# beehive-lab/GPULlama3.java

Measured on AMD Instinct MI355X. Metric: tg128 tok/s (llama-bench), Llama-3-8B Q8_0, higher is better.
Workload: dtype i8; 1 GPU; Llama-3-8B-random Q8_0 random-weight GGUF-layout model, tg128 at depth 0 (one step = 128 decode tokens, logits D2H inside the timed region); parallelism=single GPU, ranks=1, ctx=648

## Files before the change

### gpullama3.java_amd/csrc/gl3_decode_kernels.h

```cpp
#pragma once
#include <hip/hip_runtime.h>
#include <stdint.h>

#include "gl3_seqsum.h"

namespace gl3 {

constexpr int TILE_BYTES = 2176;
constexpr int MV_AUX = 4;
__host__ __device__ constexpr int mv_threads(int npw) { return 64 * (npw + MV_AUX); }

enum { PRO_RMS = 0, PRO_QUANT = 1 };
enum { EPI_STORE = 0, EPI_RESID = 1, EPI_SWIGLU = 2 };

typedef float v4f __attribute__((ext_vector_type(4)));

#ifdef GL3_MV_TIMING
__device__ long long gl3_mv_stamp[32];
#define ATT_STAMP(i) do { if (blockIdx.x == 0 && threadIdx.x == 0) gl3_mv_stamp[i] = wall_clock64(); } while (0)
#define MV_STAMP(i, cond) do { if (blockIdx.x == 0 && (cond)) gl3_mv_stamp[i] = clock64(); } while (0)
#define PV_T(...) __VA_ARGS__
#else
#define PV_T(...)
#define MV_STAMP(i, cond)
#define ATT_STAMP(i)
#endif

constexpr int TPF_MAX_PEERS = 15;
struct TpWait {
    const uint32_t* flags;
    const uint32_t* step;
    uint32_t* err;
    int mul, add, tp, me;
    unsigned spin_limit;
};
struct TpPush {
    uint32_t* ticket;
    const uint32_t* step;
    int mul, add, npeers;
    long delta[TPF_MAX_PEERS];
    uint32_t* flag[TPF_MAX_PEERS];
};
struct TpRec { TpWait w; TpPush p; };

__device__ __forceinline__ void tp_wait(const TpWait& w) {
    const uint32_t need = (__hip_atomic_load(w.step, __ATOMIC_RELAXED, __HIP_MEMORY_SCOPE_AGENT) - 1u) * (uint32_t)w.mul + (uint32_t)w.add;
    const int lane = threadIdx.x & 63;
    const bool mine = lane < w.tp && lane != w.me;
    unsigned spins = 0;
    for (;;) {
        const bool ok = !mine || (int32_t)(__hip_atomic_load(w.flags + (mine ? lane : 0), __ATOMIC_RELAXED, __HIP_MEMORY_SCOPE_SYSTEM) - need) >= 0;
        if (__builtin_amdgcn_ballot_w64(!ok) == 0) break;
        __builtin_amdgcn_s_sleep(8);
        if (++spins > w.spin_limit) { if (lane == 0) __hip_atomic_store(w.err, 1u, __ATOMIC_RELAXED, __HIP_MEMORY_SCOPE_SYSTEM); break; }
    }
    __builtin_amdgcn_fence(__ATOMIC_ACQUIRE, "");
}
__device__ __forceinline__ void tp_push_store(const TpPush& p, float* own, float v) {
    for (int j = 0; j < p.npeers; ++j)
        *reinterpret_cast<float*>(reinterpret_cast<uint8_t*>(own) + p.delta[j]) = v;
}
__device__ __forceinline__ void tp_publish(const TpPush& p, unsigned total) {
    asm volatile("s_waitcnt vmcnt(0)" ::: "memory");
    if ((threadIdx.x & 63) != 0) return;
    const unsigned ticket = __hip_atomic_fetch_add(p.ticket, 1u, __ATOMIC_RELAXED, __HIP_MEMORY_SCOPE_AGENT);
    if (ticket != total - 1) return;
    __hip_atomic_store(p.ticket, 0u, __ATOMIC_RELAXED, __HIP_MEMORY_SCOPE_AGENT);
    const uint32_t k = (__hip_atomic_load(p.step, __ATOMIC_RELAXED, __HIP_MEMORY_SCOPE_AGENT) - 1u) * (uint32_t)p.mul + (uint32_t)p.add;
    __threadfence_system();
    for (int j = 0; j < p.npeers; ++j) __hip_atomic_store(p.flag[j], k, __ATOMIC_RELEASE, __HIP_MEMORY_SCOPE_SYSTEM);
}

static __global__ __launch_bounds__(64) void tp_wait_kernel(const TpRec* r) { tp_wait(r->w); }

struct MatvecArgs {
    const uint8_t* w;
    const uint8_t* w2;
    int rows;
    int k;
    int ng;
    int nstrips;
    const float* x;
    const float* norm_w;
    float eps;
    float* out;
    const float* resid_in;
    float out_scale;
    const struct MoeSlots* moe;
    const TpRec* tp;
};

struct MoeSlots {
    const int* sel;
    size_t sel_stride;
    int x_slot_stride, out_slot_stride;
    int n_sel, sh_rows;
    const uint8_t* sh_w;
    const uint8_t* sh_w2;
    float* sh_out;
};

__device__ __forceinline__ void lds_barrier() { asm volatile("s_waitcnt lgkmcnt(0)\n\ts_barrier" ::: "memory"); }

struct LdsBarrier { __device__ __forceinline__ void operator()() const { lds_barrier(); } };

__device__ __forceinline__ float h2f(uint16_t h) { return (float)__builtin_bit_cast(_Float16, h); }

__device__ __forceinline__ float wave_max(float v) {
#pragma unroll
    for (int m = 32; m >= 1; m >>= 1) v = fmaxf(v, __shfl_xor(v, m, 64));
    return v;
}

template <bool SQ>
__device__ __forceinline__ float seq_add4(float s, const float4& a) {
    if (SQ) { s = s + a.x * a.x; s = s + a.y * a.y; s = s + a.z * a.z; s = s + a.w * a.w; }
    else { s = s + a.x; s = s + a.y; s = s + a.z; s = s + a.w; }
    return s;
}
template <bool SQ>
__device__ __forceinline__ float seq_sum_lds(const float* v, int n, float start = 0.f) {
    float s = start;
    int i = 0;
    if (n >= 16) {
        float4 a0 = *reinterpret_cast<const float4*>(v), a1 = *reinterpret_cast<const float4*>(v + 4);
        for (; i + 16 <= n; i += 8) {
            const float4 b0 = *reinterpret_cast<const float4*>(v + i + 8), b1 = *reinterpret_cast<const float4*>(v + i + 12);
            s = seq_add4<SQ>(s, a0); s = seq_add4<SQ>(s, a1);
            a0 = b0; a1 = b1;
        }
        s = seq_add4<SQ>(s, a0); s = seq_add4<SQ>(s, a1);
        i += 8;
    }
    for (; i + 4 <= n; i += 4) s = seq_add4<SQ>(s, *reinterpret_cast<const float4*>(v + i));
    for (; i < n; ++i) s = SQ ? s + v[i] * v[i] : s + v[i];
    return s;
}

__device__ __forceinline__ float mul_f32_scalar(float a, float b) {
    float r;
    asm("v_mul_f32 %0, %1, %2" : "=v"(r) : "v"(a), "v"(b));
    return r;
}

__device__ __forceinline__ float seq_sum_lds_ring(const float* v, int n, float start = 0.f) {
    float s = start;
    const int G = n >> 4;
    int i = 0;
    if (G >= 3) {
        float4 a0, a1, a2, a3, b0, b1, b2, b3, c0, c1, c2, c3;
#define SSR_LD(G_, V0_, V1_, V2_, V3_) do { const float* q_ = v + 16 * min((G_), G - 1); V0_ = *reinterpret_cast<const float4*>(q_); \
        V1_ = *reinterpret_cast<const float4*>(q_ + 4); V2_ = *reinterpret_cast<const float4*>(q_ + 8); V3_ = *reinterpret_cast<const float4*>(q_ + 12); } while (0)
#define SSR_ADD(V0_, V1_, V2_, V3_) do { s = seq_add4<false>(s, V0_); s = seq_add4<false>(s, V1_); s = seq_add4<false>(s, V2_); s = seq_add4<false>(s, V3_); } while (0)
        SSR_LD(0, a0, a1, a2, a3); SSR_LD(1, b0, b1, b2, b3); SSR_LD(2, c0, c1, c2, c3);
        int g = 0;
        for (; g + 3 <= G; g += 3) {
            SSR_ADD(a0, a1, a2, a3); SSR_LD(g + 3, a0, a1, a2, a3); __builtin_amdgcn_sched_barrier(0);
            SSR_ADD(b0, b1, b2, b3); SSR_LD(g + 4, b0, b1, b2, b3); __builtin_amdgcn_sched_barrier(0);
            SSR_ADD(c0, c1, c2, c3); SSR_LD(g + 5, c0, c1, c2, c3); __builtin_amdgcn_sched_barrier(0);
        }
        if (g < G) { SSR_ADD(a0, a1, a2, a3); ++g; }
        if (g < G) { SSR_ADD(b0, b1, b2, b3); ++g; }
#undef SSR_ADD
#undef SSR_LD
        i = 16 * G;
    }
    for (; i + 4 <= n; i += 4) s = seq_add4<false>(s, *reinterpret_cast<const float4*>(v + i));
    for (; i < n; ++i) s = s + v[i];
    return s;
}

__device__ __forceinline__ uint32_t quantize_quad_pack(float4 v, float& qs_out) {
    float amax = fmaxf(fmaxf(fabsf(v.x), fabsf(v.y)), fmaxf(fabsf(v.z), fabsf(v.w)));
    amax = fmaxf(amax, __builtin_bit_cast(float, __builtin_amdgcn_update_dpp(0, __builtin_bit_cast(int, amax), 0xB1, 0xf, 0xf, false)));
    amax = fmaxf(amax, __builtin_bit_cast(float, __builtin_amdgcn_update_dpp(0, __builtin_bit_cast(int, amax), 0x4E, 0xf, 0xf, false)));
    amax = fmaxf(amax, __builtin_bit_cast(float, __builtin_amdgcn_update_dpp(0, __builtin_bit_cast(int, amax), 0x141, 0xf, 0xf, false)));
    const float qs = amax / 127.0f;
    const float ainv = qs != 0.f ? 1.0f / qs : 0.f;
    const float s0 = v.x * ainv, s1 = v.y * ainv, s2 = v.z * ainv, s3 = v.w * ainv;
    const int q0 = (int)(s0 + copysignf(0.5f, s0)), q1 = (int)(s1 + copysignf(0.5f, s1));
    const int q2 = (int)(s2 + copysignf(0.5f, s2)), q3 = (int)(s3 + copysignf(0.5f, s3));
    qs_out = (float)(_Float16)qs;
    return (uint32_t)(q0 & 0xFF) | ((uint32_t)(q1 & 0xFF) << 8) | ((uint32_t)(q2 & 0xFF) << 16) | ((uint32_t)(q3 & 0xFF) << 24);
}

__device__ __forceinline__ void quantize_quad(float4 v, int qd, uint8_t* xq, float* xs) {
    float qs;
    const uint32_t packed = quantize_quad_pack(v, qs);
    *reinterpret_cast<uint32_t*>(xq + 4 * qd) = packed;
    if ((qd & 7) == 0) xs[qd >> 3] = qs;
}

__device__ __forceinline__ size_t bdq_offset(int qd, int tok, int tslots) {
    const int blk = qd >> 3, qi = qd & 7, c = qi >> 1;
    const int g = ((c & 1) << 1) | (c >> 1);
    return ((size_t)(blk >> 1) * tslots + tok) * 64 + 16 * g + 8 * (blk & 1) + 4 * (qi & 1);
}
__device__ __forceinline__ size_t bds_offset(int blk, int tok, int tslots) { return ((size_t)(blk >> 2) * tslots + tok) * 4 + (blk & 3); }

__device__ __forceinline__ int dot32(const int4& a0, const int4& a1, const int4& b0, const int4& b1) {
    int s = 0;
    s = __builtin_amdgcn_sdot4(a0.x, b0.x, s, false); s = __builtin_amdgcn_sdot4(a0.y, b0.y, s, false);
    s = __builtin_amdgcn_sdot4(a0.z, b0.z, s, false); s = __builtin_amdgcn_sdot4(a0.w, b0.w, s, false);
    s = __builtin_amdgcn_sdot4(a1.x, b1.x, s, false); s = __builtin_amdgcn_sdot4(a1.y, b1.y, s, false);
    s = __builtin_amdgcn_sdot4(a1.z, b1.z, s, false); s = __builtin_amdgcn_sdot4(a1.w, b1.w, s, false);
    return s;
}

template <bool NT>
__device__ __forceinline__ int4 ld16(const uint8_t* p) {
    typedef int v4i __attribute__((ext_vector_type(4)));
    v4i v;
    if (NT) v = __builtin_nontemporal_load(reinterpret_cast<const v4i*>(p));
    else v = *reinterpret_cast<const v4i*>(p);
    int4 r; r.x = v.x; r.y = v.y; r.z = v.z; r.w = v.w;
    return r;
}
template <bool NT>
__device__ __forceinline__ uint16_t ld2(const uint8_t* p) {
    if (NT) return __builtin_nontemporal_load(reinterpret_cast<const uint16_t*>(p));
    return *reinterpret_cast<const uint16_t*>(p);
}

template <int PRO, int EPI, bool NT, int NPW = 4, bool SEL = false, bool TPF = false>
__global__ __launch_bounds__(mv_threads(NPW), NPW == 4 ? 4 : 2) void matvec_q8t_kernel(const MatvecArgs a_in) {
    MatvecArgs a = a_in;
    if (SEL) {
        const int slot = blockIdx.y;
        const MoeSlots m = *a.moe;
        if (slot < m.n_sel) {
            const size_t woff = (size_t)m.sel[slot] * m.sel_stride;
            a.w += woff;
            if (a.w2) a.w2 += woff;
            a.x += (size_t)slot * m.x_slot_stride;
            a.out += (size_t)slot * m.out_slot_stride;
        } else {
            const int c = slot - m.n_sel;
            const size_t woff = (size_t)c * m.sel_stride;
            a.w = m.sh_w + woff;
            a.w2 = m.sh_w2 ? m.sh_w2 + woff : nullptr;
            a.out = m.sh_out + (size_t)c * a.rows;
            const int left = m.sh_rows - c * a.rows;
            if (left < a.rows) { a.rows = left; a.nstrips = (left + 15) / 16; }
        }
    }
    constexpr int MV_PRODUCERS = NPW;
    extern __shared__ __attribute__((aligned(16))) uint8_t smem[];
    constexpr int NM = (EPI == EPI_SWIGLU) ? 2 : 1;
    constexpr int CH = (NM == 1) ? 8 : 4;
    const int t = threadIdx.x, lane = t & 63, wave = t >> 6;
    const int nb4 = a.ng * 4;
    uint8_t* xq = smem;
    float* xs = reinterpret_cast<float*>(smem + (size_t)nb4 * 32);
    float* xf = xs + nb4;
    float* pbuf = xf + (PRO == PRO_RMS ? a.k + 32 : 0);
    float* red = pbuf + (size_t)2 * NM * a.ng * 64;
    int* sync_w = reinterpret_cast<int*>(red + 4);
    const size_t strip_bytes = (size_t)a.ng * TILE_BYTES;
    MV_STAMP(0, t == 0);
    if (t < 2) sync_w[t] = 0;

    if (wave < MV_PRODUCERS) {
        const int nt = (a.ng - wave + MV_PRODUCERS - 1) / MV_PRODUCERS;
        uint16_t sc[NM][CH];
        int4 lo[NM][CH], hi[NM][CH];
        auto issue = [&](int strip, int i0) {
#pragma unroll
            for (int u = 0; u < CH; ++u) {
                if (i0 + u < nt) {
                    const int g = wave + (i0 + u) * MV_PRODUCERS;
#pragma unroll
                    for (int m = 0; m < NM; ++m) {
                        const uint8_t* p = (m == 0 ? a.w : a.w2) + (size_t)strip * strip_bytes + (size_t)g * TILE_BYTES;
                        sc[m][u] = ld2<NT>(p + 2 * lane);
                        lo[m][u] = ld16<NT>(p + 128 + 16 * lane);
                        hi[m][u] = ld16<NT>(p + 1152 + 16 * lane);
                    }
                }
            }
        };
        auto compute = [&](int i0, float* pb) {
#pragma unroll
            for (int u = 0; u < CH; ++u) {
                if (i0 + u < nt) {
                    const int g = wave + (i0 + u) * MV_PRODUCERS;
                    const int xb = 4 * g + (lane >> 4);
                    const int4 xlo = *reinterpret_cast<const int4*>(xq + 32 * xb);
                    const int4 xhi = *reinterpret_cast<const int4*>(xq + 32 * xb + 16);
                    const float xsc = xs[xb];
#pragma unroll
                    for (int m = 0; m < NM; ++m) {
                        const int isum = dot32(lo[m][u], hi[m][u], xlo, xhi);
                        pb[(size_t)m * a.ng * 64 + g * 64 + lane] = (float)isum * (h2f(sc[m][u]) * xsc);
                    }
                }
            }
        };
        int strip = blockIdx.x;
        __syncthreads();
        if (strip < a.nstrips) issue(strip, 0);
        while (__hip_atomic_load(&sync_w[1], __ATOMIC_RELAXED, __HIP_MEMORY_SCOPE_WORKGROUP) == 0) __builtin_amdgcn_s_sleep(2);
        __builtin_amdgcn_fence(__ATOMIC_ACQUIRE, "workgroup");
        MV_STAMP(3, t == 0);
        int it = 0;
        for (; strip < a.nstrips; strip += gridDim.x, ++it) {
            float* pb = pbuf + (size_t)(it & 1) * NM * a.ng * 64;
            for (int i0 = 0; i0 < nt; i0 += CH) {
                if (it != 0 || i0 != 0) issue(strip, i0);
                compute(i0, pb);
            }
            MV_STAMP(4 + 2 * it, t == 0 && it < 4);
            __syncthreads();
            MV_STAMP(5 + 2 * it, t == 0 && it < 4);
        }
        return;
    }

    __builtin_amdgcn_s_setprio(3);
    const int ta = t - 64 * MV_PRODUCERS;
    const int nquads = a.k >> 2;
    float scale = 1.0f;
    constexpr int NXV = (PRO == PRO_RMS) ? 5 : 14;
    float4 nwv[5], xv[NXV];
    if (!TPF) {
#pragma unroll
        for (int i = 0; i < NXV; ++i) xv[i] = *reinterpret_cast<const float4*>(a.x + 4 * min(ta + 256 * i, nquads - 1));
    }
    if (PRO == PRO_RMS) {
#pragma unroll
        for (int i = 0; i < 5; ++i) nwv[i] = *reinterpret_cast<const float4*>(a.norm_w + 4 * min(ta + 256 * i, nquads - 1));
    }
    __syncthreads();
    if (TPF) {
        if (a.tp->w.flags) tp_wait(a.tp->w);
#pragma unroll
        for (int i = 0; i < NXV; ++i) xv[i] = *reinterpret_cast<const float4*>(a.x + 4 * min(ta + 256 * i, nquads - 1));
    }
    SubBarrier aux_sync{&sync_w[0], MV_AUX, 0};
    if (PRO == PRO_RMS) {
        if (nquads <= NXV * 256) {
#pragma unroll
            for (int i = 0; i < NXV; ++i) { const int qd = ta + 256 * i; if (qd < nquads) *reinterpret_cast<float4*>(xf + 4 * qd) = xv[i]; }
        } else {
            for (int qd = ta; qd < nquads; qd += 256)
                *reinterpret_cast<float4*>(xf + 4 * qd) = *reinterpret_cast<const float4*>(a.x + 4 * qd);
        }
        if (ta < 32) xf[a.k + ta] = 0.f;
        aux_sync();
        MV_STAMP(1, ta == 0);
        float ss;
        if ((size_t)2 * NM * a.ng * 64 * 4 >= ss_scratch_bytes(a.k) && a.k >= 1024 && a.k <= 5120) {
            ss = exact_sumsq_lds(xf, a.k, reinterpret_cast<uint8_t*>(pbuf), ta, aux_sync);
        } else {
            if (wave == MV_PRODUCERS) {
                const float s1 = seq_sum_lds<true>(xf, a.k);
                if (lane == 0) red[0] = s1;
            }
            aux_sync();
            ss = red[0];
        }
        MV_STAMP(2, ta == 0);
        ss /= (float)a.k;
        ss += a.eps;
        scale = (float)(1.0 / sqrt((double)ss));
    }
    for (int b = (a.k >> 5) + ta; b < nb4; b += 256) {
        xs[b] = 0.f;
        const int4 z = {0, 0, 0, 0};
        *reinterpret_cast<int4*>(xq + 32 * b) = z;
        *reinterpret_cast<int4*>(xq + 32 * b + 16) = z;
    }
    if (nquads <= NXV * 256) {
#pragma unroll
        for (int i = 0; i < NXV; ++i) {
            const int qd = ta + 256 * i;
            if (qd < nquads) {
                float4 v = xv[i];
                if (PRO == PRO_RMS) {
                    const float4 w = nwv[i];
                    v.x = w.x * (scale * v.x); v.y = w.y * (scale * v.y); v.z = w.z * (scale * v.z); v.w = w.w * (scale * v.w);
                }
                quantize_quad(v, qd, xq, xs);
            }
        }
    } else {
        for (int qd = ta; qd < nquads; qd += 256) {
            float4 v = *reinterpret_cast<const float4*>(a.x + 4 * qd);
            if (PRO == PRO_RMS) {
                const float4 w = *reinterpret_cast<const float4*>(a.norm_w + 4 * qd);
                v.x = w.x * (scale * v.x); v.y = w.y * (scale * v.y); v.z = w.z * (scale * v.z); v.w = w.w * (scale * v.w);
            }
            quantize_quad(v, qd, xq, xs);
        }
    }
    aux_sync();
    if (ta == 0) __hip_atomic_store(&sync_w[1], 1, __ATOMIC_RELEASE, __HIP_MEMORY_SCOPE_WORKGROUP);
    if (wave != MV_PRODUCERS) return;

    int it = 0;
    for (int strip = blockIdx.x; strip < a.nstrips; strip += gridDim.x, ++it) {
        __syncthreads();
        MV_STAMP(16 + 2 * it, lane == 0 && it < 4);
        const float* pb = pbuf + (size_t)(it & 1) * NM * a.ng * 64;
        v4f acc[NM];
#pragma unroll
        for (int m = 0; m < NM; ++m) acc[m] = (v4f){0.f, 0.f, 0.f, 0.f};
        int g = 0;
        for (; g + 8 <= a.ng; g += 8) {
            float av[NM][8];
#pragma unroll
            for (int m = 0; m < NM; ++m)
#pragma unroll
                for (int u = 0; u < 8; ++u) av[m][u] = pb[(size_t)m * a.ng * 64 + (g + u) * 64 + lane];
#pragma unroll
            for (int u = 0; u < 8; ++u)
#pragma unroll
                for (int m = 0; m < NM; ++m) acc[m] = __builtin_amdgcn_mfma_f32_16x16x4f32(av[m][u], 1.0f, acc[m], 0, 0, 0);
        }
        for (; g < a.ng; ++g)
#pragma unroll
            for (int m = 0; m < NM; ++m)
                acc[m] = __builtin_amdgcn_mfma_f32_16x16x4f32(pb[(size_t)m * a.ng * 64 + g * 64 + lane], 1.0f, acc[m], 0, 0, 0);
        MV_STAMP(17 + 2 * it, lane == 0 && it < 4);
        if ((lane & 15) < 4) {
            const int r = lane & 3;
            const int row = strip * 16 + 4 * (lane >> 4) + r;
            if (row < a.rows) {
                const float v0 = r == 0 ? acc[0][0] : r == 1 ? acc[0][1] : r == 2 ? acc[0][2] : acc[0][3];
                float res;
                if (EPI == EPI_STORE) res = v0 * a.out_scale;
                if (EPI == EPI_RESID) res = a.resid_in ? a.resid_in[row] + v0 * a.out_scale : v0 * a.out_scale;
                if (EPI == EPI_SWIGLU) {
                    const float v1 = r == 0 ? acc[NM - 1][0] : r == 1 ? acc[NM - 1][1] : r == 2 ? acc[NM - 1][2] : acc[NM - 1][3];
                    const float gte = v0 / (float)(1.0 + exp(-(double)v0));
                    res = gte * v1;
                }
                a.out[row] = res;
                if (TPF) tp_push_store(a.tp->p, a.out + row, res);
            }
        }
    }
    if (TPF && a.tp->p.npeers) tp_publish(a.tp->p, gridDim.x);
}

static __global__ __launch_bounds__(256) void embed_q8t_kernel(const uint8_t* __restrict__ emb, int ng, int dim,
                                                         const int* __restrict__ dyn, float* __restrict__ x, float emb_scale,
                                                         const TpRec* tp = nullptr, uint32_t* step = nullptr) {
    if (step) {
        const uint32_t s = *step;
        __syncthreads();
        if (threadIdx.x == 0) *step = s + 1;
        if (tp) {
            TpWait w = tp->w;
            const uint32_t need = s * (uint32_t)w.mul;
            const int lane = threadIdx.x & 63;
            const bool mine = lane < w.tp && lane != w.me;
            unsigned spins = 0;
            for (;;) {
                const bool ok = !mine || (int32_t)(__hip_atomic_load(w.flags + (mine ? lane : 0), __ATOMIC_RELAXED, __HIP_MEMORY_SCOPE_SYSTEM) - need) >= 0;
                if (__builtin_amdgcn_ballot_w64(!ok) == 0) break;
                __builtin_amdgcn_s_sleep(8);
                if (++spins > w.spin_limit) { if (lane == 0) __hip_atomic_store(w.err, 1u, __ATOMIC_RELAXED, __HIP_MEMORY_SCOPE_SYSTEM); break; }
            }
        }
    }
    const int token = dyn[0];
    const uint8_t* strip = emb + (size_t)(token >> 4) * ng * TILE_BYTES;
    const int i16 = token & 15;
    for (int i = threadIdx.x; i < dim; i += 256) {
        const int b = i >> 5, j = i & 31;
        const uint8_t* p = strip + (size_t)(b >> 2) * TILE_BYTES;
        const int l = i16 + 16 * (b & 3);
        const float d = h2f(*reinterpret_cast<const uint16_t*>(p + 2 * l));
        const int8_t q = (int8_t)p[(j < 16 ? 128 : 1152) + 16 * l + (j & 15)];
        x[i] = ((float)q * d) * emb_scale;
    }
}

struct AttnArgs {
    const float* qkv;
    float* kcache;
    float* vcache;
    const float* rope_cr;
    const float* rope_ci;
    const float* qnorm;
    const float* knorm;
    const float* bq;
    const float* bk;
    const float* bv;
    const int* dyn;
    float* att;
    float* xb;
    int n_heads, n_kv_heads, hs, q_dim, kv_dim, ctx;
    float eps;
    int arch;
    const int* seqv;
    const int* posv;
    size_t seq_stride;
    int qkv_stride, xb_stride;
    float att_mul;
    int win;
    int att_stride;
    float* att_t;
    float* tmax;
    float* sums;
    int group;
    uint8_t* xq_out; float* xs_out; int xq_slots;
    const TpRec* tp;
};

__device__ __forceinline__ void rope_head(float* v, int hs, const float* cr, const float* ci, int arch, int t0, int nthreads) {
    const int half = hs >> 1;
    for (int i = t0; i < half; i += nthreads) {
        const float fcr = cr[i], fci = ci[i];
        const int i0 = arch == 0 ? 2 * i : i, i1 = arch == 0 ? 2 * i + 1 : i + half;
        const float v0 = v[i0], v1 = v[i1];
        v[i0] = v0 * fcr - v1 * fci;
        v[i1] = v0 * fci + v1 * fcr;
    }
}

__device__ __forceinline__ void head_rmsnorm_wave(float* v, const float* __restrict__ w, int hs, float eps, int lane) {
    float ss = seq_sum_lds<true>(v, hs);
    ss /= (float)hs;
    ss += eps;
    ss = (float)(1.0 / sqrt((double)ss));
    for (int i = lane; i < hs; i += 64) v[i] = w[i] * (ss * v[i]);
}

constexpr int ATT_TT = 64;

static __global__ void attn_scores_kernel(const AttnArgs a) {
    extern __shared__ __attribute__((aligned(16))) float sm[];
    const int hs = a.hs, kvmul = a.n_heads / a.n_kv_heads, half = hs >> 1;
    float* q_s = sm;
    float* kt = q_s + kvmul * hs;
    float* cr_s = kt + ATT_TT * (hs + 4);
    float* ci_s = cr_s + half;
    const int t = threadIdx.x, nthr = blockDim.x;
    const int sp = blockIdx.x, kvh = blockIdx.y;
    const int pos = a.dyn[1];
    const int t0 = sp * ATT_TT;
    if (t0 > pos) return;
    const int t1 = min(pos + 1, t0 + ATT_TT);
    const bool owns_pos = (t1 == pos + 1);
    const int pitch = hs + 4;
    float* krow = kt + (pos - t0) * pitch;
    const int q4 = hs >> 2;
    const int nrows_cache = owns_pos ? (t1 - 1 - t0) : (t1 - t0);
    const int nk4 = nrows_cache * q4;
    constexpr int KMAX = 16;
    float4 kreg[KMAX];
    const int per = (nk4 + nthr - 1) / nthr;
#pragma unroll
    for (int u = 0; u < KMAX; ++u) {
        kreg[u] = make_float4(0.f, 0.f, 0.f, 0.f);
        if (u < per) {
            const int i = min(t + u * nthr, nk4 - 1);
            kreg[u] = *reinterpret_cast<const float4*>(a.kcache + (size_t)(t0 + i / q4) * a.kv_dim + kvh * hs + 4 * (i % q4));
        }
    }
    for (int i = t; i < kvmul * hs; i += nthr) q_s[i] = a.bq ? a.qkv[(kvh * kvmul) * hs + i] + a.bq[(kvh * kvmul) * hs + i] : a.qkv[(kvh * kvmul) * hs + i];
    for (int i = t; i < half; i += nthr) { cr_s[i] = a.rope_cr[(size_t)pos * half + i]; ci_s[i] = a.rope_ci[(size_t)pos * half + i]; }
    float vraw[4] = {0.f, 0.f, 0.f, 0.f};
    if (owns_pos) {
        for (int i = t; i < hs; i += nthr) krow[i] = a.bk ? a.qkv[a.q_dim + kvh * hs + i] + a.bk[kvh * hs + i] : a.qkv[a.q_dim + kvh * hs + i];
#pragma unroll
        for (int u = 0; u < 4; ++u) {
            const int i = t + u * nthr;
            if (i < hs) vraw[u] = a.bv ? a.qkv[a.q_dim + a.kv_dim + kvh * hs + i] + a.bv[kvh * hs + i] : a.qkv[a.q_dim + a.kv_dim + kvh * hs + i];
        }
    }
    if (per > KMAX) {
        for (int i = t; i < nk4; i += nthr) {
            const float4 v = *reinterpret_cast<const float4*>(a.kcache + (size_t)(t0 + i / q4) * a.kv_dim + kvh * hs + 4 * (i % q4));
            *reinterpret_cast<float4*>(kt + (i / q4) * pitch + 4 * (i % q4)) = v;
        }
    } else {
#pragma unroll
        for (int u = 0; u < KMAX; ++u) {
            const int i = t + u * nthr;
            if (u < per && i < nk4) *reinterpret_cast<float4*>(kt + (i / q4) * pitch + 4 * (i % q4)) = kreg[u];
        }
    }
    __syncthreads();
    if (a.arch == 1) {
        const int nvec = kvmul + (owns_pos ? 1 : 0);
        for (int vec = t >> 6; vec < nvec; vec += nthr >> 6)
            head_rmsnorm_wave(vec < kvmul ? q_s + vec * hs : krow, vec < kvmul ? a.qnorm : a.knorm, hs, a.eps, t & 63);
        __syncthreads();
    }
    for (int h = 0; h < kvmul; ++h) rope_head(q_s + h * hs, hs, cr_s, ci_s, a.arch, t, nthr);
    if (owns_pos) rope_head(krow, hs, cr_s, ci_s, a.arch, t, nthr);
    __syncthreads();
    if (owns_pos) {
#pragma unroll
        for (int u = 0; u < 4; ++u) {
            const int i = t + u * nthr;
            if (i < hs) {
                a.kcache[(size_t)pos * a.kv_dim + kvh * hs + i] = krow[i];
                a.vcache[(size_t)pos * a.kv_dim + kvh * hs + i] = vraw[u];
            }
        }
    }
    const int hq = t >> 6, r = t & 63;
    float my_score = -INFINITY;
    if (hq < kvmul && t0 + r < t1) {
        const float* q = q_s + hq * hs;
        const float* kk = kt + r * pitch;
        float score = 0.f;
        float4 qv = *reinterpret_cast<const float4*>(q), kv = *reinterpret_cast<const float4*>(kk);
        for (int j = 4; j < hs; j += 4) {
            const float4 qn = *reinterpret_cast<const float4*>(q + j), kn = *reinterpret_cast<const float4*>(kk + j);
            score = score + qv.x * kv.x; score = score + qv.y * kv.y; score = score + qv.z * kv.z; score = score + qv.w * kv.w;
            qv = qn; kv = kn;
        }
        score = score + qv.x * kv.x; score = score + qv.y * kv.y; score = score + qv.z * kv.z; score = score + qv.w * kv.w;
        const float sqrt_hs = (float)sqrt((double)hs);
        my_score = a.att_mul != 0.f ? score * a.att_mul : score / sqrt_hs;
        a.att[(size_t)(kvh * kvmul + hq) * a.att_stride + t0 + r] = my_score;
    }
    if (a.tmax && hq < kvmul) {
        const float m = wave_max(my_score);
        if (r == 0) a.tmax[(size_t)(kvh * kvmul + hq) * gridDim.x + sp] = m;
    }
}

constexpr int SCL_WGS = 32, SCL_LOADERS = 4;
template <int HS>
static __global__ __launch_bounds__(64 * (4 + SCL_LOADERS), 1) void attn_scores_loop_kernel(const AttnArgs a, int n_tiles_max) {
    extern __shared__ __attribute__((aligned(16))) float sm[];
    constexpr int hs = HS, half = HS / 2, pitch = HS + 4, q4 = HS / 4;
    const int kvmul = a.n_heads / a.n_kv_heads;
    float* q_s = sm;
    float* kt = q_s + kvmul * hs;
    float* krow_s = kt + 2 * ATT_TT * pitch;
    float* cr_s = krow_s + hs;
    float* ci_s = cr_s + half;
    const int t = threadIdx.x, nthr = blockDim.x;
    const int wave = __builtin_amdgcn_readfirstlane(t >> 6);
    const int w = blockIdx.x, kvh = blockIdx.y;
    const int pos = a.dyn[1];
    const int ntile = pos / ATT_TT + 1;
    if (w >= ntile) return;
    const int cnt = (ntile - w + SCL_WGS - 1) / SCL_WGS;
    const bool owner = ((ntile - 1) % SCL_WGS) == w;
    for (int i = t; i < kvmul * hs; i += nthr) q_s[i] = a.bq ? a.qkv[(kvh * kvmul) * hs + i] + a.bq[(kvh * kvmul) * hs + i] : a.qkv[(kvh * kvmul) * hs + i];
    for (int i = t; i < half; i += nthr) { cr_s[i] = a.rope_cr[(size_t)pos * half + i]; ci_s[i] = a.rope_ci[(size_t)pos * half + i]; }
    float vraw = 0.f;
    if (owner && t < hs) {
        krow_s[t] = a.bk ? a.qkv[a.q_dim + kvh * hs + t] + a.bk[kvh * hs + t] : a.qkv[a.q_dim + kvh * hs + t];
        vraw = a.bv ? a.qkv[a.q_dim + a.kv_dim + kvh * hs + t] + a.bv[kvh * hs + t] : a.qkv[a.q_dim + a.kv_dim + kvh * hs + t];
    }
    __syncthreads();
    if (a.arch == 1) {
        const int nvec = kvmul + (owner ? 1 : 0);
        for (int vec = wave; vec < nvec; vec += nthr >> 6) head_rmsnorm_wave(vec < kvmul ? q_s + vec * hs : krow_s, vec < kvmul ? a.qnorm : a.knorm, hs, a.eps, t & 63);
        __syncthreads();
    }
    for (int h = 0; h < kvmul; ++h) rope_head(q_s + h * hs, hs, cr_s, ci_s, a.arch, t, nthr);
    if (owner) rope_head(krow_s, hs, cr_s, ci_s, a.arch, t, nthr);
    __syncthreads();
    if (owner && t < hs) {
        a.kcache[(size_t)pos * a.kv_dim + kvh * hs + t] = krow_s[t];
        a.vcache[(size_t)pos * a.kv_dim + kvh * hs + t] = vraw;
    }
    if (wave >= kvmul) {
        if (wave >= kvmul + SCL_LOADERS) return;
        const int lt = t - 64 * kvmul;
        constexpr int PER = ATT_TT * q4 / (64 * SCL_LOADERS);
#define SCL_DECL(S_) float4 S_##0 = {0.f, 0.f, 0.f, 0.f}, S_##1 = S_##0, S_##2 = S_##0, S_##3 = S_##0, S_##4 = S_##0, S_##5 = S_##0, S_##6 = S_##0, S_##7 = S_##0
        SCL_DECL(k0_); SCL_DECL(k1_); SCL_DECL(k2_);
#undef SCL_DECL
        const float* kb = a.kcache + (size_t)kvh * hs;
#define SCL_LOAD1(S_, U_, T0_) do { if ((U_) < PER) { const int p_ = lt + 256 * (U_), row_ = max(min((T0_) + p_ / q4, pos - 1), 0); \
            S_##U_ = *reinterpret_cast<const float4*>(kb + (size_t)row_ * a.kv_dim + 4 * (p_ % q4)); } } while (0)
#define SCL_LOAD(S_, I_) do { \
            const int t0_ = (w + min((I_), cnt - 1) * SCL_WGS) * ATT_TT; \
            SCL_LOAD1(S_, 0, t0_); SCL_LOAD1(S_, 1, t0_); SCL_LOAD1(S_, 2, t0_); SCL_LOAD1(S_, 3, t0_); \
            SCL_LOAD1(S_, 4, t0_); SCL_LOAD1(S_, 5, t0_); SCL_LOAD1(S_, 6, t0_); SCL_LOAD1(S_, 7, t0_); \
        } while (0)
#define SCL_STORE1(S_, U_, KD_) do { if ((U_) < PER) { const int p_ = lt + 256 * (U_); \
            if (st0_ + p_ / q4 < pos) *reinterpret_cast<float4*>((KD_) + (p_ / q4) * pitch + 4 * (p_ % q4)) = S_##U_; } } while (0)
#define SCL_STORE(S_, I_) do { \
            float* kd_ = kt + ((I_) & 1) * ATT_TT * pitch; \
            const int st0_ = (w + (I_) * SCL_WGS) * ATT_TT; \
            SCL_STORE1(S_, 0, kd_); SCL_STORE1(S_, 1, kd_); SCL_STORE1(S_, 2, kd_); SCL_STORE1(S_, 3, kd_); \
            SCL_STORE1(S_, 4, kd_); SCL_STORE1(S_, 5, kd_); SCL_STORE1(S_, 6, kd_); SCL_STORE1(S_, 7, kd_); \
            if (owner && (I_) == cnt - 1 && lt < q4)         \
                *reinterpret_cast<float4*>(kd_ + (pos & (ATT_TT - 1)) * pitch + 4 * lt) = *reinterpret_cast<const float4*>(krow_s + 4 * lt); \
        } while (0)
#define SCL_STEP(S_, I_) do { \
            if ((I_) < cnt) {                                \
                PV_T(const long long s0_ = clock64();) \
                SCL_STORE(S_, (I_)); \
                PV_T(const long long b0_ = clock64(); lst_ += b0_ - s0_;) \
                lds_barrier(); \
                PV_T(lbw_ += clock64() - b0_;) \
            } \
            SCL_LOAD(S_, (I_) + 3);                          \
        } while (0)
        PV_T(long long lst_ = 0, lbw_ = 0; const long long lts_ = clock64();)
        SCL_LOAD(k0_, 0); SCL_LOAD(k1_, 1); SCL_LOAD(k2_, 2);
        for (int i = 0; i < cnt; i += 3) { SCL_STEP(k0_, i); SCL_STEP(k1_, i + 1); SCL_STEP(k2_, i + 2); }
        PV_T(if (blockIdx.x == 0 && blockIdx.y == 0 && lt == 0) { gl3_mv_stamp[8] = lst_; gl3_mv_stamp[9] = lbw_; gl3_mv_stamp[10] = clock64() - lts_; })
#undef SCL_LOAD
#undef SCL_LOAD1
#undef SCL_STORE
#undef SCL_STORE1
#undef SCL_STEP
        return;
    }
    const int hq = wave, r = t & 63;
    const float sqrt_hs = (float)sqrt((double)hs);
    const float4* q4p = reinterpret_cast<const float4*>(q_s + hq * hs);
    PV_T(long long cbw_ = 0; const long long cts_ = clock64();)
    for (int i = 0; i < cnt; ++i) {
        const int sp = w + i * SCL_WGS, t0 = sp * ATT_TT, t1 = min(pos + 1, t0 + ATT_TT);
        PV_T(const long long cb0_ = clock64();)
        lds_barrier();
        PV_T(cbw_ += clock64() - cb0_;)
        const float4* kk4 = reinterpret_cast<const float4*>(kt + (i & 1) * ATT_TT * pitch + r * pitch);
        float score = 0.f;
        float4 qa[4], ka[4], qb[4], kb[4];
#define SCL_RD(Q_, K_, Q0_) do { _Pragma("unroll") for (int u = 0; u < 4; ++u) { Q_[u] = q4p[(Q0_) + u]; K_[u] = kk4[(Q0_) + u]; } } while (0)
#define SCL_USE(Q_, K_) do { _Pragma("unroll") for (int u = 0; u < 4; ++u) { \
            score = score + mul_f32_scalar(Q_[u].x, K_[u].x); score = score + mul_f32_scalar(Q_[u].y, K_[u].y); \
            score = score + mul_f32_scalar(Q_[u].z, K_[u].z); score = score + mul_f32_scalar(Q_[u].w, K_[u].w); } } while (0)
        SCL_RD(qa, ka, 0);
#pragma unroll
        for (int g = 0; g < HS / 16; g += 2) {
            SCL_RD(qb, kb, 4 * (g + 1));
            __builtin_amdgcn_sched_barrier(0);
            SCL_USE(qa, ka);
            __builtin_amdgcn_sched_barrier(0);
            if (g + 2 < HS / 16) SCL_RD(qa, ka, 4 * (g + 2));
            __builtin_amdgcn_sched_barrier(0);
            SCL_USE(qb, kb);
            __builtin_amdgcn_sched_barrier(0);
        }
#undef SCL_RD
#undef SCL_USE
        float my_score = -INFINITY;
        if (t0 + r < t1) {
// ... 602 lines not shown
```

Before: 470.0 tok/s.

## Stream matvec producer loads across strips and overlap reduction with per-wave progress flags

Producer waves now run a continuous software pipeline of tile loads that spans strip boundaries, and prefetch the quantized activation for the next tile in double-buffered registers. The reducing wave no longer waits on a full workgroup barrier before each strip. It polls per-wave progress counters in LDS and starts MFMA accumulation on groups of 8 tiles as soon as they are ready. The aim is to hide load latency at strip edges and let reduction overlap with producer compute, at the cost of spin-polling and more complex synchronization (lds_barrier pairing) that could deadlock or race if miscounted. Timing stamps are also extended to multiple workgroups under the debug flag.

After: 476.7 tok/s (median of 6 runs). 1.4% higher.

```diff
diff --git a/gpullama3.java_amd/csrc/gl3_decode_kernels.h b/gpullama3.java_amd/csrc/gl3_decode_kernels.h
--- a/gpullama3.java_amd/csrc/gl3_decode_kernels.h
+++ b/gpullama3.java_amd/csrc/gl3_decode_kernels.h
@@ -18,7 +18,9 @@
 #ifdef GL3_MV_TIMING
 __device__ long long gl3_mv_stamp[32];
 #define ATT_STAMP(i) do { if (blockIdx.x == 0 && threadIdx.x == 0) gl3_mv_stamp[i] = wall_clock64(); } while (0)
-#define MV_STAMP(i, cond) do { if (blockIdx.x == 0 && (cond)) gl3_mv_stamp[i] = clock64(); } while (0)
+constexpr int MV_STAMP_WGS = 64;
+__device__ long long gl3_mv_wg_stamp[MV_STAMP_WGS][32];
+#define MV_STAMP(i, cond) do { if ((blockIdx.x & 7) == 0 && (blockIdx.x >> 3) < MV_STAMP_WGS && blockIdx.y == 0 && (cond)) gl3_mv_wg_stamp[blockIdx.x >> 3][i] = clock64(); } while (0)
 #define PV_T(...) __VA_ARGS__
 #else
 #define PV_T(...)
@@ -256,63 +258,82 @@
     float* pbuf = xf + (PRO == PRO_RMS ? a.k + 32 : 0);
     float* red = pbuf + (size_t)2 * NM * a.ng * 64;
     int* sync_w = reinterpret_cast<int*>(red + 4);
+    int* prog = sync_w + 4;
     const size_t strip_bytes = (size_t)a.ng * TILE_BYTES;
     MV_STAMP(0, t == 0);
-    if (t < 2) sync_w[t] = 0;
+    if (t < 4 + MV_PRODUCERS) sync_w[t] = 0;
 
     if (wave < MV_PRODUCERS) {
         const int nt = (a.ng - wave + MV_PRODUCERS - 1) / MV_PRODUCERS;
+        const int strip0 = blockIdx.x;
+        const int nmine = strip0 < a.nstrips ? (a.nstrips - strip0 + (int)gridDim.x - 1) / (int)gridDim.x : 0;
+        __syncthreads();
+        if (nt == 0) {
+            for (int n = 0; n < nmine; ++n) lds_barrier();
+            return;
+        }
+        const int total = nmine * nt;
+        const int rounds = (total + CH - 1) / CH;
         uint16_t sc[NM][CH];
         int4 lo[NM][CH], hi[NM][CH];
-        auto issue = [&](int strip, int i0) {
-#pragma unroll
-            for (int u = 0; u < CH; ++u) {
-                if (i0 + u < nt) {
-                    const int g = wave + (i0 + u) * MV_PRODUCERS;
-#pragma unroll
-                    for (int m = 0; m < NM; ++m) {
-                        const uint8_t* p = (m == 0 ? a.w : a.w2) + (size_t)strip * strip_bytes + (size_t)g * TILE_BYTES;
-                        sc[m][u] = ld2<NT>(p + 2 * lane);
-                        lo[m][u] = ld16<NT>(p + 128 + 16 * lane);
-                        hi[m][u] = ld16<NT>(p + 1152 + 16 * lane);
-                    }
-                }
-            }
+        int is = strip0, ii = 0;
+        auto issue = [&](int u) {
+            const bool valid = is < a.nstrips;
+            const size_t off = valid ? (size_t)is * strip_bytes + (size_t)(wave + ii * MV_PRODUCERS) * TILE_BYTES : (size_t)0;
+            const int ln = valid ? lane : 0;
+#pragma unroll
+            for (int m = 0; m < NM; ++m) {
+                const uint8_t* p = (m == 0 ? a.w : a.w2) + off;
+                sc[m][u] = ld2<NT>(p + 2 * ln);
+                lo[m][u] = ld16<NT>(p + 128 + 16 * ln);
+                hi[m][u] = ld16<NT>(p + 1152 + 16 * ln);
+            }
+            if (++ii == nt) { ii = 0; is += gridDim.x; }
         };
-        auto compute = [&](int i0, float* pb) {
-#pragma unroll
-            for (int u = 0; u < CH; ++u) {
-                if (i0 + u < nt) {
-                    const int g = wave + (i0 + u) * MV_PRODUCERS;
-                    const int xb = 4 * g + (lane >> 4);
-                    const int4 xlo = *reinterpret_cast<const int4*>(xq + 32 * xb);
-                    const int4 xhi = *reinterpret_cast<const int4*>(xq + 32 * xb + 16);
-                    const float xsc = xs[xb];
-#pragma unroll
-                    for (int m = 0; m < NM; ++m) {
-                        const int isum = dot32(lo[m][u], hi[m][u], xlo, xhi);
-                        pb[(size_t)m * a.ng * 64 + g * 64 + lane] = (float)isum * (h2f(sc[m][u]) * xsc);
-                    }
-                }
-            }
+        int ci = 0, it = 0, done = 0;
+        float* pb = pbuf;
+        int4 xlo[2], xhi[2];
+        float xsc[2];
+        auto xread = [&](int tile, int par) {
+            const int xb = 4 * (wave + tile * MV_PRODUCERS) + (lane >> 4);
+            xlo[par] = *reinterpret_cast<const int4*>(xq + 32 * xb);
+            xhi[par] = *reinterpret_cast<const int4*>(xq + 32 * xb + 16);
+            xsc[par] = xs[xb];
         };
-        int strip = blockIdx.x;
-        __syncthreads();
-        if (strip < a.nstrips) issue(strip, 0);
+        auto dot = [&](int u) {
+            const int g = wave + ci * MV_PRODUCERS;
+            xread(ci + 1 == nt ? 0 : ci + 1, (u + 1) & 1);
+#pragma unroll
+            for (int m = 0; m < NM; ++m) {
+                const int isum = dot32(lo[m][u], hi[m][u], xlo[u & 1], xhi[u & 1]);
+                pb[(size_t)m * a.ng * 64 + g * 64 + lane] = (float)isum * (h2f(sc[m][u]) * xsc[u & 1]);
+            }
+            ++done;
+            asm volatile("" ::: "memory");
+            if (lane == 0) __hip_atomic_store(&prog[wave], done, __ATOMIC_RELAXED, __HIP_MEMORY_SCOPE_WORKGROUP);
+            MV_STAMP(12, t == 0 && done == 1);
+            if (++ci == nt) {
+                ci = 0;
+                MV_STAMP(4 + 2 * it, t == 0 && it < 4);
+                lds_barrier();
+                MV_STAMP(5 + 2 * it, t == 0 && it < 4);
+                ++it;
+                pb = pbuf + (size_t)(it & 1) * NM * a.ng * 64;
+            }
+        };
+#pragma unroll
+        for (int u = 0; u < CH; ++u) issue(u);
         while (__hip_atomic_load(&sync_w[1], __ATOMIC_RELAXED, __HIP_MEMORY_SCOPE_WORKGROUP) == 0) __builtin_amdgcn_s_sleep(2);
         __builtin_amdgcn_fence(__ATOMIC_ACQUIRE, "workgroup");
         MV_STAMP(3, t == 0);
-        int it = 0;
-        for (; strip < a.nstrips; strip += gridDim.x, ++it) {
-            float* pb = pbuf + (size_t)(it & 1) * NM * a.ng * 64;
-            for (int i0 = 0; i0 < nt; i0 += CH) {
-                if (it != 0 || i0 != 0) issue(strip, i0);
-                compute(i0, pb);
-            }
-            MV_STAMP(4 + 2 * it, t == 0 && it < 4);
-            __syncthreads();
-            MV_STAMP(5 + 2 * it, t == 0 && it < 4);
-        }
+        xread(0, 0);
+        for (int r = 0; r + 1 < rounds; ++r) {
+#pragma unroll
+            for (int u = 0; u < CH; ++u) { dot(u); issue(u); }
+        }
+        const int left = rounds ? total - (rounds - 1) * CH : 0;
+#pragma unroll
+        for (int u = 0; u < CH; ++u) if (u < left) dot(u);
         return;
     }
 
@@ -397,16 +418,27 @@
     if (ta == 0) __hip_atomic_store(&sync_w[1], 1, __ATOMIC_RELEASE, __HIP_MEMORY_SCOPE_WORKGROUP);
     if (wave != MV_PRODUCERS) return;
 
+    const int ntw = lane < MV_PRODUCERS ? (a.ng - lane + MV_PRODUCERS - 1) / MV_PRODUCERS : 0;
+    int have = 0;
     int it = 0;
     for (int strip = blockIdx.x; strip < a.nstrips; strip += gridDim.x, ++it) {
-        __syncthreads();
-        MV_STAMP(16 + 2 * it, lane == 0 && it < 4);
+        auto await = [&](int gend) {
+            const int need = it * ntw + (lane < MV_PRODUCERS && gend > lane ? (gend - lane + MV_PRODUCERS - 1) / MV_PRODUCERS : 0);
+            while (__builtin_amdgcn_ballot_w64(have < need) != 0) {
+                have = __hip_atomic_load(&prog[lane < MV_PRODUCERS ? lane : 0], __ATOMIC_RELAXED, __HIP_MEMORY_SCOPE_WORKGROUP);
+                if (__builtin_amdgcn_ballot_w64(have < need) == 0) break;
+                __builtin_amdgcn_s_sleep(1);
+            }
+            __builtin_amdgcn_fence(__ATOMIC_ACQUIRE, "workgroup");
+        };
         const float* pb = pbuf + (size_t)(it & 1) * NM * a.ng * 64;
         v4f acc[NM];
 #pragma unroll
         for (int m = 0; m < NM; ++m) acc[m] = (v4f){0.f, 0.f, 0.f, 0.f};
         int g = 0;
         for (; g + 8 <= a.ng; g += 8) {
+            await(g + 8);
+            MV_STAMP(16 + 2 * it, lane == 0 && it < 4 && g == 0);
             float av[NM][8];
 #pragma unroll
             for (int m = 0; m < NM; ++m)
@@ -416,12 +448,17 @@
             for (int u = 0; u < 8; ++u)
 #pragma unroll
                 for (int m = 0; m < NM; ++m) acc[m] = __builtin_amdgcn_mfma_f32_16x16x4f32(av[m][u], 1.0f, acc[m], 0, 0, 0);
+        }
+        if (g < a.ng) {
+            await(a.ng);
+            MV_STAMP(16 + 2 * it, lane == 0 && it < 4 && g == 0);
         }
         for (; g < a.ng; ++g)
 #pragma unroll
             for (int m = 0; m < NM; ++m)
                 acc[m] = __builtin_amdgcn_mfma_f32_16x16x4f32(pb[(size_t)m * a.ng * 64 + g * 64 + lane], 1.0f, acc[m], 0, 0, 0);
         MV_STAMP(17 + 2 * it, lane == 0 && it < 4);
+        lds_barrier();
         if ((lane & 15) < 4) {
             const int r = lane & 3;
             const int row = strip * 16 + 4 * (lane >> 4) + r;
@@ -440,6 +477,7 @@
             }
         }
     }
+    MV_STAMP(25, lane == 0);
     if (TPF && a.tp->p.npeers) tp_publish(a.tp->p, gridDim.x);
 }
 
```
